# Quyans/GOI-Hyperplane

Hardware: AMD Instinct MI355X
Metric: training views/sec (rasterizer fwd+bwd), 1M Gaussians @1600x1056 RGB+16-d feat (higher is better)
Workload: dtype f32

## Files before the change

goi_hyperplane_amd/build.py:

```python
from __future__ import annotations

import os
import subprocess
import sys
from concurrent.futures import ThreadPoolExecutor

HERE = os.path.dirname(os.path.abspath(__file__))
ROOT = os.path.dirname(HERE)
CSRC = os.path.join(HERE, "csrc")
LIBDIR = os.path.join(HERE, "lib")
LIB = os.path.join(LIBDIR, "libgoi_raster.so")
HIPCC = os.environ.get("HIPCC", "/opt/rocm/bin/hipcc")
ARCH = "gfx950"

COMMON = ["--offload-arch=" + ARCH] + os.environ.get("GOI_EXTRA_FLAGS", "").split() + ["-O3", "-std=c++17", "-fPIC", "-I" + os.path.join(ROOT, "include"), "-I" + CSRC,
          "-munsafe-fp-atomics", "-Wall", "-Wno-unused-function"]
UNITS = {
    "api.hip": [],
    "scan_sort.hip": [],
    "preprocess.hip": ["-ffp-contract=off"],
    "binning.hip": [],
    "reduce_rows.hip": [],
    "render_fwd.hip": ["-fno-slp-vectorize"],
    "blend_stats.hip": [],
    "render_bwd.hip": [],
    "render_bwd_tile.hip": [],
    "render_bwd_sem.hip": [],
    "semantic_head.hip": [],
    "knn.hip": ["-ffp-contract=off"],
    "adam.hip": ["-ffp-contract=off"],
    "codebook_loss.hip": [],
    "osh.hip": [],
    "dbscan.hip": ["-ffp-contract=off"],
    "masks.hip": [],
    "codebook_init.hip": [],
    "photometric.hip": [],
    "densify.hip": ["-ffp-contract=off"],
    "display.hip": ["-ffp-contract=off"],
    "pca.hip": ["-ffp-contract=off"],
    "field.hip": ["-ffp-contract=off"],
    "mesh.hip": ["-ffp-contract=off"],
    "texture.hip": ["-ffp-contract=off"],
    "edit.hip": ["-ffp-contract=off"],
}


EXT = os.path.join(LIBDIR, "_goi_C.so")
EXT_SRC = os.path.join(CSRC, "torch_binding.cpp")


def build_torch_binding(force: bool = False, verbose: bool = False) -> str:
    import sysconfig
    import torch
    hdr = os.path.join(ROOT, "include", "goi_raster.h")
    if not force and os.path.exists(EXT) and all(os.path.getmtime(f) <= os.path.getmtime(EXT) for f in (EXT_SRC, hdr, LIB)):
        return EXT
    tdir = os.path.dirname(torch.__file__)
    cmd = [os.environ.get("CXX", "g++"), "-O2", "-std=c++17", "-fPIC", "-shared", "-D__HIP_PLATFORM_AMD__=1",
           "-DUSE_ROCM=1", "-DTORCH_EXTENSION_NAME=_goi_C", "-DTORCH_API_INCLUDE_EXTENSION_H",
           f"-D_GLIBCXX_USE_CXX11_ABI={int(torch._C._GLIBCXX_USE_CXX11_ABI)}",
           "-I" + os.path.join(tdir, "include"), "-I" + os.path.join(tdir, "include", "torch", "csrc", "api", "include"),
           "-I" + sysconfig.get_paths()["include"], "-I/opt/rocm/include", "-I" + os.path.join(ROOT, "include"),
           EXT_SRC, "-o", EXT, "-L" + os.path.join(tdir, "lib"), "-ltorch", "-ltorch_cpu", "-ltorch_python", "-lc10",
           "-lc10_hip", "-ltorch_hip", "-L" + LIBDIR, "-lgoi_raster", "-Wl,-rpath,$ORIGIN"]
    if verbose:
        print(" ".join(cmd))
    subprocess.check_call(cmd)
    return EXT


def _newer(src: str, dst: str) -> bool:
    return (not os.path.exists(dst)) or os.path.getmtime(src) > os.path.getmtime(dst)


def build(force: bool = False, verbose: bool = False) -> str:
    os.makedirs(LIBDIR, exist_ok=True)
    objdir = os.path.join(HERE, "build")
    os.makedirs(objdir, exist_ok=True)
    headers = [os.path.join(CSRC, h) for h in os.listdir(CSRC) if h.endswith(".h")] + [
        os.path.join(ROOT, "include", "goi_raster.h")]
    hdr_time = max(os.path.getmtime(h) for h in headers)

    def compile_one(item):
        name, extra = item
        src = os.path.join(CSRC, name)
        obj = os.path.join(objdir, name + ".o")
        if force or _newer(src, obj) or hdr_time > os.path.getmtime(obj):
            cmd = [HIPCC] + COMMON + extra + ["-c", src, "-o", obj]
            if verbose:
                print(" ".join(cmd))
            subprocess.check_call(cmd)
            return obj, True
        return obj, False

    with ThreadPoolExecutor(max_workers=4) as ex:
        results = list(ex.map(compile_one, UNITS.items()))
    objs = [o for o, _ in results]
    if force or any(c for _, c in results) or not os.path.exists(LIB):
        cmd = [HIPCC, "--offload-arch=" + ARCH, "-shared", "-fPIC", "-o", LIB] + objs
        if verbose:
            print(" ".join(cmd))
        subprocess.check_call(cmd)
    try:
        build_torch_binding(force=force, verbose=verbose)
    except Exception as ex:
        import warnings
        if os.path.exists(EXT):
            os.remove(EXT)
        warnings.warn(f"the compiled torch binding (_goi_C.so) could not be built: {ex}; goi_hyperplane_amd._C falls back "
                      "to its ctypes binding of the same C ABI (same kernels, ~0.14 ms more host time per step)")
    return LIB


if __name__ == "__main__":
    print(build(force="--force" in sys.argv, verbose=True))
```

goi_hyperplane_amd/csrc/render_bwd.hip:

```cpp
#include "blend_common.h"

namespace goi {

namespace {


#if !defined(GOI_BWD_WAVES)
#define GOI_BWD_WAVES 4
#endif
#define GOI_BWD_LAUNCH_BOUNDS __launch_bounds__(64, (S4 <= 4 ? GOI_BWD_WAVES : 2))

#ifndef GOI_TSTRIDE
#define GOI_TSTRIDE 66
#endif
constexpr int GROUP = 8;
constexpr int BATCH = 32;
constexpr int TSTRIDE = GOI_TSTRIDE;

template <int S4>
struct BwdCfg {
    static constexpr int NF4 = 1 + S4;
    static constexpr int NSEM = 4 * S4;
    static constexpr int NCH = NSEM + 4;
    static constexpr int NB = (NSEM + 15) / 16;
};

template <int S4, bool F16, bool MASKS>
__global__ GOI_BWD_LAUNCH_BOUNDS void render_bwd_rows_k(
    const uint2* __restrict__ ranges, const uint32_t* __restrict__ point_list, int W, int H, int gx, int gy,
    int n_quads, int S, const GaussRec* __restrict__ rec, const float* __restrict__ semantics,
    const int* __restrict__ radii, const uint4* __restrict__ aux, const float* __restrict__ bg,
    const float* __restrict__ out_alpha, const uint32_t* __restrict__ n_contrib, const float* __restrict__ dL_dpix,
    const float* __restrict__ dL_dpixsem, const float* __restrict__ dL_dpixdepth, const float* __restrict__ dL_dalphas,
    float* __restrict__ rows, uint8_t* __restrict__ flags, int row_floats,
    const uint32_t* __restrict__ counters, const uint32_t* __restrict__ qorder,
    const unsigned long long* __restrict__ qmask0, const unsigned long long* __restrict__ qmask,
    const uint32_t* __restrict__ qcost) {
    using Cfg = BwdCfg<S4>;
    const bool cull = counters[COUNTER_CULL] != 0;
    constexpr int NF4 = Cfg::NF4, NSEM = Cfg::NSEM, NCH = Cfg::NCH, NB = Cfg::NB;
    __shared__ f32x4 s_geo[BATCH + GROUP];
    __shared__ f32x4 s_geo2[BATCH + GROUP];
    __shared__ float2 s_cen[BATCH + GROUP];
    __shared__ __attribute__((aligned(16))) float4 s_feat[BATCH * NF4];
    constexpr int TS = TSTRIDE;
    constexpr int T_BYTES = F16 ? F16_FLOATS * 4 : 2 * GROUP * TSTRIDE * 4;
    __shared__ __attribute__((aligned(16))) char s_traw[T_BYTES];
    float* const s_t = reinterpret_cast<float*>(s_traw);

    const QuadGeom t = quad_geom_of(qorder ? (int)qorder[quad_slot()] : quad_slot(), W, H, gx, n_quads);
    if (t.tile < 0) return;
    if (counters[COUNTER_OVF]) return;
    const int lane = t.lane;
    const uint2 range = ranges[t.tile];
    const size_t HW = (size_t)W * H;
    const size_t pix_id = (size_t)W * t.py + t.px;
    const size_t pix_ld = t.inside ? pix_id : 0;
    const uint32_t nc_ld = n_contrib[pix_ld];
    const float oa_ld = out_alpha[pix_ld];
    float dLch[NCH];
    if (dL_dpixsem && S == NSEM) {
#pragma unroll
        for (int ch = 0; ch < NSEM; ch++) dLch[ch] = dL_dpixsem[ch * HW + pix_ld];
    } else {
#pragma unroll
        for (int ch = 0; ch < NSEM; ch++) dLch[ch] = (dL_dpixsem && ch < S) ? dL_dpixsem[ch * HW + pix_ld] : 0.f;
    }
    dLch[NSEM + 0] = dL_dpix ? dL_dpix[0 * HW + pix_ld] : 0.f;
    dLch[NSEM + 1] = dL_dpix ? dL_dpix[1 * HW + pix_ld] : 0.f;
    dLch[NSEM + 2] = dL_dpix ? dL_dpix[2 * HW + pix_ld] : 0.f;
    dLch[NSEM + 3] = dL_dpixdepth ? dL_dpixdepth[pix_ld] : 0.f;
    float dLa = dL_dalphas ? dL_dalphas[pix_ld] : 0.f;

    const int last_contributor = t.inside ? (int)nc_ld : 0;
    const int n_proc = qcost ? (int)qcost[__builtin_amdgcn_readfirstlane(4 * t.tile + t.q)] : wave_max_i32(last_contributor);
    if (n_proc == 0) return;
    const int rounds = (n_proc + BATCH - 1) / BATCH;

    const float T_final = t.inside ? (1.f - oa_ld) : 0.f;
    float T = T_final;
    if (!t.inside) {
#pragma unroll
        for (int ch = 0; ch < NCH; ch++) dLch[ch] = 0.f;
        dLa = 0.f;
    }
    const float bg_dot = bg[0] * dLch[NSEM] + bg[1] * dLch[NSEM + 1] + bg[2] * dLch[NSEM + 2];
    float R = 0.f;
    f32x2 dL2[NCH / 2];
#pragma unroll
    for (int i = 0; i < NCH / 2; i++) dL2[i] = f32x2{dLch[2 * i], dLch[2 * i + 1]};
    const f32x4* s_feat4 = reinterpret_cast<const f32x4*>(s_feat);

    const int kq = lane >> 4, mm = lane & 15;
    float bfrag[F16 ? 1 : NB][F16 ? 1 : 16];
    float bmix[F16 ? 1 : 16];
    f16x8 Wh[F16 ? NB : 1][2], Wl[F16 ? NB : 1][2], Cc[2];
    float unscale[F16 ? NB : 1], unscale_c = 0.f;
    bf16x8 Bas;
    constexpr int BT = 17;
    static_assert(64 * BT * 4 <= F16_FLOATS * 4 && 64 * 16 * 4 <= T_BYTES, "staging region too small");
    const float k1 = mm == 4 ? 1.f : 0.f, ku = mm == 5 ? 1.f : 0.f, kv = mm == 6 ? 1.f : 0.f;
    const float kuu = mm == 7 ? 1.f : 0.f, kuv = mm == 8 ? 1.f : 0.f, kvv = mm == 9 ? 1.f : 0.f;
    auto basis = [&](int p) {
        const float u = (float)(p & 7) - 3.5f, v = (float)(p >> 3) - 3.5f;
        return k1 + ku * u + kv * v + kuu * (u * u) + kuv * (u * v) + kvv * (v * v);
    };
    if constexpr (F16) {
#pragma unroll
        for (int nb = 0; nb < NB; nb++) {
#pragma unroll
            for (int c = 0; c < 16; c++) {
                const int ch = nb * 16 + c;
                s_t[lane * BT + c] = ch < NSEM ? dLch[ch] : 0.f;
            }
            __builtin_amdgcn_wave_barrier();
            float y[2][8];
#pragma unroll
            for (int c2 = 0; c2 < 2; c2++)
#pragma unroll
                for (int i = 0; i < 8; i++) y[c2][i] = s_t[(32 * c2 + 8 * kq + i) * BT + mm];
            f16_b_operand(y, Wh[nb], Wl[nb], unscale[nb]);
            __builtin_amdgcn_wave_barrier();
        }
        {
#pragma unroll
            for (int c = 0; c < 4; c++) s_t[lane * 5 + c] = dLch[NSEM + c];
            __builtin_amdgcn_wave_barrier();
            float y[2][8];
#pragma unroll
            for (int c2 = 0; c2 < 2; c2++)
#pragma unroll
                for (int i = 0; i < 8; i++) y[c2][i] = s_t[(32 * c2 + 8 * kq + i) * 5 + (mm & 3)];
            f16x8 hi[2], lo[2];
            f16_b_operand(y, hi, lo, unscale_c);
            typedef uint32_t u32x4 __attribute__((ext_vector_type(4)));
#pragma unroll
            for (int c2 = 0; c2 < 2; c2++) {
                const u32x4 hu = __builtin_bit_cast(u32x4, hi[c2]), lu = __builtin_bit_cast(u32x4, lo[c2]);
                u32x4 cu;
#pragma unroll
                for (int i = 0; i < 4; i++) cu[i] = mm < 4 ? hu[i] : mm < 8 ? lu[i] : 0u;
                Cc[c2] = __builtin_bit_cast(f16x8, cu);
            }
            __builtin_amdgcn_wave_barrier();
        }
        {
            float y[8];
            const float vb = (float)kq - 1.5f;
#pragma unroll
            for (int i = 0; i < 8; i++) {
                const float u = (float)i - 3.5f;
                y[i] = mm == 0 ? 1.f : mm == 1 ? u : mm == 2 ? vb : mm == 3 ? u * u : mm == 4 ? u * vb : mm == 5 ? vb * vb : 0.f;
            }
            bf16x8 unused;
            split_pack8(y, Bas, unused);
        }
    } else {
#pragma unroll
        for (int nb = 0; nb < NB; nb++) {
#pragma unroll
            for (int c = 0; c < 16; c++) {
                const int ch = nb * 16 + c;
                s_t[lane * 16 + c] = ch < NSEM ? dLch[ch] : 0.f;
            }
            __builtin_amdgcn_wave_barrier();
#pragma unroll
            for (int s = 0; s < 16; s++) bfrag[nb][s] = s_t[(4 * s + kq) * 16 + mm];
            __builtin_amdgcn_wave_barrier();
        }
#pragma unroll
        for (int c = 0; c < 4; c++) s_t[lane * 4 + c] = dLch[NSEM + c];
        __builtin_amdgcn_wave_barrier();
#pragma unroll
        for (int s = 0; s < 16; s++) bmix[s] = mm < 4 ? s_t[(4 * s + kq) * 4 + mm] : basis(4 * s + kq);
        __builtin_amdgcn_wave_barrier();
    }
    auto uniform = [](float x) { return __int_as_float(__builtin_amdgcn_readfirstlane(__float_as_int(x))); };
    const float QCX = uniform(t.QX0 + 3.5f), QCY = uniform(t.QY0 + 3.5f);
    const f32x2 uv = {t.pxf - QCX, t.pyf - QCY};
    const float half_W = uniform(0.5f * W), half_H = uniform(0.5f * H);

    uint32_t id_n = 0;
    unsigned long long w_n = 0;
    float4 q0_n = make_float4(0, 0, 0, 0), q1_n = make_float4(1.f, 0.f, -1.f, -1.f);
    const int tile_u = __builtin_amdgcn_readfirstlane(t.tile), q_u = __builtin_amdgcn_readfirstlane(t.q);
    const uint32_t x0_u = (uint32_t)__builtin_amdgcn_readfirstlane((int)range.x);
    auto prefetch = [&](int b) {
        if constexpr (MASKS) {
            w_n = *member_mask_ptr(const_cast<unsigned long long*>(qmask0), const_cast<unsigned long long*>(qmask), tile_u, q_u,
                                   x0_u, b >> 1);
            const int pos = b * BATCH + lane;
            if (lane < BATCH && pos < n_proc) id_n = point_list[range.x + (uint32_t)pos];
        } else {
            const int k = b * BATCH + lane;
            q1_n.z = -1.f;
            if (lane < BATCH && k < n_proc) {
                id_n = point_list[range.x + (n_proc - 1 - k)];
                const float4* r4 = reinterpret_cast<const float4*>(rec + id_n);
                q0_n = r4[0];
                q1_n = r4[1];
            }
        }
    };
    prefetch(MASKS ? rounds - 1 : 0);

    int nslot = 0;
    unsigned long long jpack = 0;

    auto xrow = [](int rho) { return rho * 8 + 16 * (rho >> 3); };
    auto flush_group = [&](int cnt) {
        f32x4 acc[NB];
        f32x4 accx = {0.f, 0.f, 0.f, 0.f};
#pragma unroll
        for (int nb = 0; nb < NB; nb++) acc[nb] = f32x4{0.f, 0.f, 0.f, 0.f};
        __builtin_amdgcn_wave_barrier();
        if constexpr (F16) {
            const f32x4* wsrc = reinterpret_cast<const f32x4*>(s_t + f16_lane_offset(mm, kq));
            {
                const f32x4* src = wsrc + (f16_row(GROUP) - f16_row(0)) / 4;
                const f32x4 a0 = src[0], a1 = src[1];
                const float y[8] = {a0.x, a0.y, a0.z, a0.w, a1.x, a1.y, a1.z, a1.w};
                bf16x8 Hh, Hl, Ht;
                split3_pack8(y, Hh, Hl, Ht);
                accx = __builtin_amdgcn_mfma_f32_16x16x32_bf16(Ht, Bas, accx, 0, 0, 0);
                accx = __builtin_amdgcn_mfma_f32_16x16x32_bf16(Hl, Bas, accx, 0, 0, 0);
                accx = __builtin_amdgcn_mfma_f32_16x16x32_bf16(Hh, Bas, accx, 0, 0, 0);
            }
            f32x4 accc = {0.f, 0.f, 0.f, 0.f};
            {
                f16x8 A0, A1;
                f16_a_operands(wsrc, A0, A1);
#pragma unroll
                for (int nb = 0; nb < NB; nb++) {
                    acc[nb] = __builtin_amdgcn_mfma_f32_16x16x32_f16(A0, Wl[nb][0], acc[nb], 0, 0, 0);
                    acc[nb] = __builtin_amdgcn_mfma_f32_16x16x32_f16(A1, Wl[nb][1], acc[nb], 0, 0, 0);
                    acc[nb] = __builtin_amdgcn_mfma_f32_16x16x32_f16(A0, Wh[nb][0], acc[nb], 0, 0, 0);
                    acc[nb] = __builtin_amdgcn_mfma_f32_16x16x32_f16(A1, Wh[nb][1], acc[nb], 0, 0, 0);
                }
                accc = __builtin_amdgcn_mfma_f32_16x16x32_f16(A0, Cc[0], accc, 0, 0, 0);
                accc = __builtin_amdgcn_mfma_f32_16x16x32_f16(A1, Cc[1], accc, 0, 0, 0);
            }
            __builtin_amdgcn_wave_barrier();
            if (mm < 8) {
                float* xb = s_t + xrow(4 * kq) + mm;
#pragma unroll
                for (int r = 0; r < 4; r++) xb[8 * r] = accx[r];
            }
            f32x2 sem[NB];
#pragma unroll
            for (int nb = 0; nb < NB; nb++) sem[nb] = (acc[nb].xy + acc[nb].zw) * unscale[nb];
            f32x2 col = accc.xy + accc.zw;
            col.x += __int_as_float(__builtin_amdgcn_update_dpp(0, __float_as_int(col.x), 0x104, 0xF, 0xF, true));
            col.y += __int_as_float(__builtin_amdgcn_update_dpp(0, __float_as_int(col.y), 0x104, 0xF, 0xF, true));
            col *= unscale_c;
#pragma unroll
            for (int e = 0; e < 2; e++) {
                const int j = 2 * kq + e;
                if (j < cnt) {
                    const int idx = (int)((jpack >> (8 * j)) & 0xFF);
                    float* dst = rows + (size_t)__float_as_uint(s_geo2[idx].w) * row_floats;
#pragma unroll
                    for (int nb = 0; nb < NB; nb++) {
                        const int ch = nb * 16 + mm;
                        if (ch < NSEM) dst[ch] = sem[nb][e];
                    }
                    if (mm < 4) dst[NSEM + mm] = col[e];
                }
            }
        } else {
#pragma unroll
            for (int s = 0; s < 16; s++) {
                const float a = s_t[mm * TS + 4 * s + kq];
#pragma unroll
                for (int nb = 0; nb < NB; nb++)
                    acc[nb] = __builtin_amdgcn_mfma_f32_16x16x4f32(a, bfrag[nb][s], acc[nb], 0, 0, 0);
                accx = __builtin_amdgcn_mfma_f32_16x16x4f32(a, bmix[s], accx, 0, 0, 0);
            }
        }
        __builtin_amdgcn_wave_barrier();
#pragma unroll
        for (int r = 0; r < 4 && !F16; r++) {
            const int row = 4 * kq + r;
            if (row >= GROUP && mm >= 4 && mm < 12) s_t[(row - GROUP) * 8 + (mm - 4)] = accx[r];
            if (row < cnt) {
                const int idx = (int)((jpack >> (8 * row)) & 0xFF);
                float* dst = rows + (size_t)__float_as_uint(s_geo2[idx].w) * row_floats;
#pragma unroll
                for (int nb = 0; nb < NB; nb++) {
                    const int ch = nb * 16 + mm;
                    if (ch < NSEM) dst[ch] = acc[nb][r];
                }
                if (mm < 4) dst[NSEM + mm] = accx[r];
            }
        }
        __builtin_amdgcn_wave_barrier();
        if (lane < cnt) {
            const float4 m03 = *reinterpret_cast<const float4*>(&s_t[lane * 8]);
            const float2 m45 = *reinterpret_cast<const float2*>(&s_t[lane * 8 + 4]);
            const int idx = (int)((jpack >> (8 * lane)) & 0xFF);
            const f32x4 g = s_geo[idx];
            const f32x4 g2 = s_geo2[idx];
            const float2 cen = s_cen[idx];
            const uint32_t slot = __float_as_uint(g2.w);
            const float Dx = cen.x, Dy = cen.y;
            float ca, cb, cc, inv_o;
            coef_decode(g, g2, ca, cb, cc, inv_o);
            float m0, sx, sy, sxx, sxy, syy;
            auto shift = [&](const float4& a, const float2& b, float DX, float DY) {
                m0 += a.x;
                sx += DX * a.x - a.y;
                sy += DY * a.x - a.z;
                sxx += DX * DX * a.x - 2.f * DX * a.y + a.w;
                sxy += DX * DY * a.x - DX * a.z - DY * a.y + b.x;
                syy += DY * DY * a.x - 2.f * DY * a.z + b.y;
            };
            m0 = sx = sy = sxx = sxy = syy = 0.f;
            if constexpr (F16) {
                const int r1 = 4 * (lane >> 1) + (lane & 1);
                shift(*reinterpret_cast<const float4*>(&s_t[xrow(r1)]), *reinterpret_cast<const float2*>(&s_t[xrow(r1) + 4]), Dx, Dy + 2.f);
                shift(*reinterpret_cast<const float4*>(&s_t[xrow(r1 + 2)]), *reinterpret_cast<const float2*>(&s_t[xrow(r1 + 2) + 4]), Dx, Dy - 2.f);
            } else {
                shift(m03, m45, Dx, Dy);
            }
            float* dst = rows + (size_t)slot * row_floats + NCH;
            dst[0] = -half_W * (ca * sx + cb * sy);
            dst[1] = -half_H * (cc * sy + cb * sx);
            dst[2] = -0.5f * sxx;
            dst[3] = -0.5f * sxy;
            dst[4] = -0.5f * syy;
            dst[5] = m0 * inv_o;
            flags[slot] = 1;
        }
        __builtin_amdgcn_wave_barrier();
    };

    for (int bi = 0; bi < rounds; bi++) {
        const int b = MASKS ? rounds - 1 - bi : bi;
        const uint32_t id = id_n;
        float4 q0 = q0_n, q1 = q1_n;
        bool hit;
        unsigned long long m;
        if constexpr (MASKS) {
            const uint32_t mem = (uint32_t)__builtin_amdgcn_readfirstlane((int)(uint32_t)(w_n >> (32 * (b & 1))));
            m = mem;
            hit = lane < BATCH && ((mem >> lane) & 1u);
            if (bi + 1 < rounds) prefetch(b - 1);
        } else {
            hit = ellipse_hits_quadrant(q0.x, q0.y, q0.z, q0.w, q1.x, q1.y, q1.z, q1.w, t.QX0, t.QY0);
            if (bi + 1 < rounds) prefetch(b + 1);
            m = __ballot(hit);
        }
        if (m == 0) continue;
        if (hit) {
            const float4* r4 = reinterpret_cast<const float4*>(rec + id);
            const float* srow = semantics + (size_t)id * S;
            const bool rows_of_float4 = (S & 3) == 0;
            lds_dma16(r4 + 2, &s_feat[0]);
            if (rows_of_float4) {
#pragma unroll
                for (int i = 0; i < S4; i++)
                    lds_dma16(reinterpret_cast<const float4*>(srow) + i, &s_feat[(1 + i) * BATCH]);
            }
            if constexpr (MASKS) {
                q0 = r4[0];
                q1 = r4[1];
            }
            int x0, y0, x1, y1;
            const uint4 ax = aux[id];
            listed_rect(q0.x, q0.y, (int)ax.y, q1.z, q1.w, cull, gx, gy, x0, y0, x1, y1);
            const uint32_t inst = ax.x + tile_instance(aux_mask(ax), t.tx, t.ty, x0, y0, x1);
            const PolyCoef pc = poly_coefs(q0.x, q0.y, q0.z, q0.w, q1.x, q1.y, QCX, QCY);
            int sl = lane;
            asm volatile("" : "+v"(sl));
            s_geo[sl] = f32x4{pc.A35.x, pc.A35.y, pc.A12.x, pc.A12.y};
            s_geo2[sl] = f32x4{pc.A0, pc.A4, pc.lim, __uint_as_float(inst * 4u + (uint32_t)t.q)};
            s_cen[sl] = make_float2(q0.x - QCX, q0.y - QCY);
            if (!rows_of_float4) {
#pragma unroll
                for (int i = 0; i < S4; i++) {
                    float4 v;
                    v.x = (4 * i + 0 < S) ? srow[4 * i + 0] : 0.f;
                    v.y = (4 * i + 1 < S) ? srow[4 * i + 1] : 0.f;
                    v.z = (4 * i + 2 < S) ? srow[4 * i + 2] : 0.f;
                    v.w = (4 * i + 3 < S) ? srow[4 * i + 3] : 0.f;
                    s_feat[(1 + i) * BATCH + sl] = v;
                }
            }
        }
        __builtin_amdgcn_s_waitcnt(0x0F70);
        __builtin_amdgcn_wave_barrier();

        while (m) {
            int j, pos0;
            if constexpr (MASKS) {
                j = 31 - __builtin_clz((uint32_t)m);
                m &= ~(1ull << j);
                pos0 = b * BATCH + j;
            } else {
                j = __builtin_ctzll(m);
                m &= m - 1;
                pos0 = n_proc - 1 - (b * BATCH + j);
            }
            const f32x4 g = s_geo[j];
            const f32x4 g2 = s_geo2[j];
            const PairEval e = eval_poly(g.xy, g.zw, g2.x, g2.y, g2.z, uv);
            const bool live = pos0 < last_contributor;
            if constexpr (!MASKS)
                if (!any_all(live, e.below, e.seen)) continue;
            const bool c = live && e.hit;

            const f32x4 f0 = s_feat4[j];
            f32x2 da = f0.xy * dL2[NSEM / 2];
            f32x2 db = f0.zw * dL2[NSEM / 2 + 1];
#pragma unroll
            for (int i = 0; i < S4; i++) {
                const f32x4 f = s_feat4[(1 + i) * BATCH + j];
                da = __builtin_elementwise_fma(f.xy, dL2[2 * i], da);
                db = __builtin_elementwise_fma(f.zw, dL2[2 * i + 1], db);
            }
            const f32x2 dot2 = da + db;
            const float dotv = (dot2.x + dot2.y) + dLa;
            const float one_m_a = 1.f - e.alpha;
            const float inv = __builtin_amdgcn_rcpf(one_m_a);
            const float Tn = T * inv;
            float wgt = 0.f, hval = 0.f;
            if (c) {
                const float dL_dopa = (dotv - R) * Tn - (T_final * inv) * bg_dot;
                R = e.alpha * dotv + one_m_a * R;
                T = Tn;
                wgt = e.alpha * Tn;
                hval = e.E * dL_dopa;
            }
            if constexpr (F16) {
                const int wrow = nslot * 72 + ((nslot & 1) << 2);
                s_t[wrow + lane] = wgt;
                s_t[wrow + lane + (f16_row(GROUP) - f16_row(0))] = hval;
            } else {
                s_t[nslot * TS + lane] = wgt;
                s_t[(GROUP + nslot) * TS + lane] = hval;
            }
            jpack |= (unsigned long long)j << (8 * nslot);
            nslot++;
            if (nslot == GROUP) {
                flush_group(GROUP);
                nslot = 0;
                jpack = 0;
            }
        }
        __builtin_amdgcn_wave_barrier();
        if (nslot > 0 && bi + 1 < rounds) {
            const int idx = (int)((jpack >> (8 * (lane & 7))) & 0xFF);
            if (lane < nslot) {
                s_geo[BATCH + lane] = s_geo[idx];
                s_geo2[BATCH + lane] = s_geo2[idx];
                s_cen[BATCH + lane] = s_cen[idx];
            }
            constexpr unsigned long long CARRY = 0x0706050403020100ull + 0x0101010101010101ull * BATCH;
            jpack = CARRY & ((1ull << (8 * nslot)) - 1ull);
            __builtin_amdgcn_wave_barrier();
        }
    }
    if (nslot > 0) flush_group(nslot);
}

constexpr int QO_THREADS = 1024, QO_WAVES = QO_THREADS / 64, QO_BUCKETS = 64, QO_ROUNDS = 16;
constexpr int QO_CLEAR_BLOCKS = 248;
__global__ __launch_bounds__(QO_THREADS) void quad_order_k(const uint32_t* __restrict__ qcost, int n_quads, int per,
                                                           uint32_t* __restrict__ qorder, int shift,
                                                           uint8_t* __restrict__ clear_flags,
                                                           const uint32_t* __restrict__ n_dev, uint32_t cap,
                                                           uint32_t* __restrict__ clear_ctl) {
    if (blockIdx.x >= 8) {
        if (clear_ctl && blockIdx.x == 8 && threadIdx.x < 8) clear_ctl[threadIdx.x] = 0u;
        if (!clear_flags) return;
        const size_t nq = ((size_t)min(*n_dev, cap) * 4 + 15) / 16;
        uint4* dst = reinterpret_cast<uint4*>(clear_flags);
        for (size_t i = (size_t)(blockIdx.x - 8) * QO_THREADS + threadIdx.x; i < nq; i += (size_t)QO_CLEAR_BLOCKS * QO_THREADS)
            dst[i] = make_uint4(0u, 0u, 0u, 0u);
        return;
    }
    __shared__ uint32_t cnt[QO_WAVES][QO_BUCKETS];
    const int band = blockIdx.x, base = band * per;
    const int n = max(0, min(per, n_quads - base));
    const int lane = threadIdx.x & 63, w = threadIdx.x >> 6;
    for (int i = threadIdx.x; i < QO_WAVES * QO_BUCKETS; i += QO_THREADS) (&cnt[0][0])[i] = 0;
    __syncthreads();
    const int chunk = (per + QO_WAVES - 1) / QO_WAVES;
    const unsigned long long lt = (1ull << lane) - 1ull;
    uint32_t d_r[QO_ROUNDS], rank_r[QO_ROUNDS];
#pragma unroll
    for (int r = 0; r < QO_ROUNDS; r++) {
        if (r * 64 >= chunk) break;
        const int e = w * chunk + r * 64 + lane;
        const bool ok = r * 64 + lane < chunk && e < n;
        const uint32_t c = ok ? qcost[base + e] : 0u;
        const uint32_t d = (uint32_t)(QO_BUCKETS - 1) - min((uint32_t)(QO_BUCKETS - 1), c >> shift);
        unsigned long long peers = __ballot(ok);
#pragma unroll
        for (int b = 0; b < 6; b++) {
            const bool bit = (d >> b) & 1u;
            const unsigned long long bal = __ballot(bit);
            peers &= bit ? bal : ~bal;
        }
        const uint32_t prev = ok ? cnt[w][d] : 0u;
        const uint32_t below = (uint32_t)__popcll(peers & lt);
        d_r[r] = d;
        rank_r[r] = prev + below;
        __builtin_amdgcn_wave_barrier();
        if (ok && below == 0) cnt[w][d] = prev + (uint32_t)__popcll(peers);
        __builtin_amdgcn_wave_barrier();
    }
    __syncthreads();
    if (threadIdx.x < 64) {
        uint32_t tot = 0;
        for (int ww = 0; ww < QO_WAVES; ww++) tot += cnt[ww][lane];
        uint32_t incl = tot;
#pragma unroll
        for (int dd = 1; dd < 64; dd <<= 1) {
            const uint32_t o = __shfl_up(incl, dd, 64);
            if (lane >= dd) incl += o;
        }
        uint32_t run = incl - tot;
        for (int ww = 0; ww < QO_WAVES; ww++) {
            const uint32_t t = cnt[ww][lane];
            cnt[ww][lane] = run;
            run += t;
        }
    }
    __syncthreads();
#pragma unroll
    for (int r = 0; r < QO_ROUNDS; r++) {
        const int e = w * chunk + r * 64 + lane;
        if (r * 64 + lane < chunk && e < n) qorder[base + cnt[w][d_r[r]] + rank_r[r]] = (uint32_t)(base + e);
    }
    for (int i = n + threadIdx.x; i < per; i += QO_THREADS) qorder[base + i] = 0xFFFFFFFFu;
}

template <int S4>
void launch_bwd_rows_s4(const GoiRasterScene& sc, const GeomView& g, const ImageView& im, const uint32_t* point_list,
                        const int* radii, const float* out_alpha, const PixelGrads& dpix, const BwdScratchView& scr,
                        bool exact_flush, bool walk_masks, hipStream_t s, const unsigned long long* qmask) {
    const int gx = (sc.W + TILE - 1) / TILE, gy = (sc.H + TILE - 1) / TILE;
    const int n_quads = gx * gy * 4;
#define GOI_LAUNCH_ROWS(F16, MASKS)                                                                                    \
    render_bwd_rows_k<S4, F16, MASKS><<<dim3(quad_grid(n_quads)), dim3(64), 0, s>>>(                                     \
        im.ranges, point_list, sc.W, sc.H, gx, gy, n_quads, sc.S, g.rec, sc.semantics, radii, g.aux, sc.bg, out_alpha, \
        im.n_contrib, dpix.color, dpix.semantic, dpix.depth, dpix.alpha, scr.rows, scr.flags, bwd_row_floats(sc.S),    \
        g.counters, quad_order_enabled(sc.W, sc.H) ? im.qorder : nullptr, im.qmask0, qmask, im.qcost)
    const bool masks = qmask != nullptr && walk_masks;
    if (exact_flush) {
        if (masks) GOI_LAUNCH_ROWS(false, true);
        else GOI_LAUNCH_ROWS(false, false);
    } else {
        if (masks) GOI_LAUNCH_ROWS(true, true);
        else GOI_LAUNCH_ROWS(true, false);
    }
#undef GOI_LAUNCH_ROWS
}

}

bool quad_order_enabled(int W, int H) {
    const int gx = (W + TILE - 1) / TILE, gy = (H + TILE - 1) / TILE;
    const int per = quad_grid(gx * gy * 4) / 8;
    return g_options.bwd_order != 0 && (per + QO_WAVES - 1) / QO_WAVES <= 64 * QO_ROUNDS;
}

bool launch_quad_order(const GoiRasterScene& sc, const ImageView& im, hipStream_t s, uint8_t* clear_flags,
                       const uint32_t* n_dev, uint32_t cap, uint32_t* clear_ctl) {
    if (!quad_order_enabled(sc.W, sc.H)) return false;
    const int gx = (sc.W + TILE - 1) / TILE, gy = (sc.H + TILE - 1) / TILE;
    const int n_quads = gx * gy * 4, per = quad_grid(n_quads) / 8;
    quad_order_k<<<dim3(clear_flags ? 8 + QO_CLEAR_BLOCKS : 8), dim3(QO_THREADS), 0, s>>>(
        im.qcost, n_quads, per, im.qorder, 3 + g_options.bwd_order, clear_flags, n_dev, cap, clear_ctl);
    return true;
}

void launch_render_bwd_rows(const GoiRasterScene& sc, const GeomView& g, const ImageView& im, const uint32_t* point_list,
                            const int* radii, const float* out_alpha, const PixelGrads& dpix, const BwdScratchView& scr,
                            bool exact_flush, bool walk_masks, hipStream_t s, const unsigned long long* qmask) {
#define GOI_CALL(N) launch_bwd_rows_s4<N>(sc, g, im, point_list, radii, out_alpha, dpix, scr, exact_flush, walk_masks, s, qmask)
    GOI_DISPATCH_S4(sc.S, GOI_CALL)
#undef GOI_CALL
}

}
```

goi_hyperplane_amd/csrc/render_fwd.hip:

```cpp
#include "blend_common.h"

namespace goi {

namespace {

template <int S4, bool TRACE, bool UNROLL2, bool MASKS, bool LEARN = false>
__global__ __launch_bounds__(64) void render_fwd_k(const uint2* __restrict__ ranges,
                                                   const uint32_t* __restrict__ point_list, int W, int H, int gx,
                                                   int n_quads, int S, const GaussRec* __restrict__ rec,
                                                   const float* __restrict__ semantics, const float* __restrict__ bg,
                                                   float* __restrict__ out_color, float* __restrict__ out_sem,
                                                   float* __restrict__ out_depth, float* __restrict__ out_alpha,
                                                   uint32_t* __restrict__ n_contrib, const float* __restrict__ img_sem,
                                                   float* __restrict__ gau_sem, int* __restrict__ num_gsem,
                                                   uint32_t* __restrict__ qcost, unsigned long long* __restrict__ qmask0,
                                                   unsigned long long* __restrict__ qmask, const float* __restrict__ zcut,
                                                   uint32_t* __restrict__ zlearn, uint32_t* __restrict__ frame_flags,
                                                   uint32_t* __restrict__ host_words, uint32_t stamp) {
    constexpr int NF4 = TRACE ? 1 : 1 + S4;
    constexpr int NSEM = TRACE ? 0 : 4 * S4;
    __shared__ f32x4 s_geo[64];
    __shared__ f32x4 s_geo2[64];
    __shared__ float4 s_feat[64 * NF4];
    const f32x4* s_feat4 = reinterpret_cast<const f32x4*>(s_feat);
    __shared__ uint32_t s_id[TRACE ? 64 : 1];

    if (host_words && blockIdx.x == 0 && threadIdx.x < 32) {
        host_words[threadIdx.x] = (frame_flags - COUNTER_OVF)[threadIdx.x];
        __threadfence_system();
        if (threadIdx.x == 0 && stamp)
            __hip_atomic_store(&host_words[HOST_STAMP_WORD], stamp, __ATOMIC_RELEASE, __HIP_MEMORY_SCOPE_SYSTEM);
    }
    const QuadGeom t = quad_geom(W, H, gx, n_quads);
    if (t.tile < 0) return;
    const int tq = quad_slot();
    const uint2 range = ranges[t.tile];
    const float QCX = t.QX0 + 3.5f, QCY = t.QY0 + 3.5f;
    const f32x2 uv = {t.pxf - QCX, t.pyf - QCY};
    const int len = (int)(range.y - range.x);
    const int rounds = (len + 63) / 64;
    const size_t HW = (size_t)W * H;
    const size_t pix_id = (size_t)W * t.py + t.px;
    const int lane = t.lane;

    float T = 1.0f;
    float T_live = t.inside ? 1.0f : 0.0f;
    auto all_done = [&]() { return __builtin_amdgcn_ballot_w64(T_live != 0.0f) == 0; };
    uint32_t last_contributor = 0;
    uint32_t stop_pos = 0;
    f32x2 C2[2] = {{0.f, 0.f}, {0.f, 0.f}};
    f32x2 Cs2[NSEM > 0 ? NSEM / 2 : 1];
#pragma unroll
    for (int i = 0; i < NSEM / 2; i++) Cs2[i] = f32x2{0.f, 0.f};

    uint32_t id_n = 0;
    float4 q0_n = make_float4(0, 0, 0, 0), q1_n = make_float4(1.f, 0.f, -1.f, -1.f), q2_n = make_float4(0, 0, 0, 0);
    auto prefetch = [&](int b) {
        const int k = b * 64 + lane;
        q1_n.z = -1.f;
        if (k < len) {
            id_n = point_list[range.x + k];
            const float4* r4 = reinterpret_cast<const float4*>(rec + id_n);
            q0_n = r4[0];
            q1_n = r4[1];
            q2_n = r4[2];
        }
    };
    if (rounds > 0) prefetch(0);

    const int tile_u = __builtin_amdgcn_readfirstlane(t.tile), q_u = __builtin_amdgcn_readfirstlane(t.q);
    const uint32_t x0_u = (uint32_t)__builtin_amdgcn_readfirstlane((int)range.x);
    auto store_members = [&](int b, unsigned long long mm) {
        if constexpr (MASKS)
            if (lane == 0) *member_mask_ptr(qmask0, qmask, tile_u, q_u, x0_u, b) = mm;
    };
    int b_end = rounds;
    for (int b = 0; b < rounds; b++) {
        if (all_done()) {
            b_end = b;
            break;
        }
        unsigned long long members = 0;
        const uint32_t id = id_n;
        const float4 q0 = q0_n, q1 = q1_n, q2 = q2_n;
        const bool hit = ellipse_hits_quadrant(q0.x, q0.y, q0.z, q0.w, q1.x, q1.y, q1.z, q1.w, t.QX0, t.QY0);
        if (b + 1 < rounds) prefetch(b + 1);
        unsigned long long m = __ballot(hit);
        if (m != 0 && hit) {
            const PolyCoef pc = poly_coefs(q0.x, q0.y, q0.z, q0.w, q1.x, q1.y, QCX, QCY);
            s_geo[lane] = f32x4{pc.A35.x, pc.A35.y, pc.A12.x, pc.A12.y};
            s_geo2[lane] = f32x4{pc.A0, pc.A4, pc.lim, 0.f};
            s_feat[lane * NF4] = q2;
            if constexpr (TRACE) {
                s_id[lane] = id;
            } else {
                const float* srow = semantics + (size_t)id * S;
                if ((S & 3) == 0) {
#pragma unroll
                    for (int i = 0; i < S4; i++) s_feat[lane * NF4 + 1 + i] = reinterpret_cast<const float4*>(srow)[i];
                } else {
#pragma unroll
                    for (int i = 0; i < S4; i++) {
                        float4 v;
                        v.x = (4 * i + 0 < S) ? srow[4 * i + 0] : 0.f;
                        v.y = (4 * i + 1 < S) ? srow[4 * i + 1] : 0.f;
                        v.z = (4 * i + 2 < S) ? srow[4 * i + 2] : 0.f;
                        v.w = (4 * i + 3 < S) ? srow[4 * i + 3] : 0.f;
                        s_feat[lane * NF4 + 1 + i] = v;
                    }
                }
            }
        }
        __builtin_amdgcn_wave_barrier();

        auto apply = [&](int j, const PairEval& e, bool valid) {
            const float test_T = T_live * (1.f - e.alpha);
            const bool c0 = valid && e.hit;
            const bool ok = test_T >= kTMin;
            const bool c = c0 && ok;
            const bool some = any_all(e.below, e.seen, ok);
            if (valid && some) {
                if constexpr (MASKS) asm("s_bitset1_b64 %0, %1" : "+s"(members) : "s"(j));
                const float wgt = c ? e.alpha * T_live : 0.f;
                const f32x2 w2 = {wgt, wgt};
                const f32x4 f0 = s_feat4[j * NF4];
                C2[0] = __builtin_elementwise_fma(f0.xy, w2, C2[0]);
                C2[1] = __builtin_elementwise_fma(f0.zw, w2, C2[1]);
                if constexpr (!TRACE) {
#pragma unroll
                    for (int i = 0; i < S4; i++) {
                        const f32x4 f = s_feat4[j * NF4 + 1 + i];
                        Cs2[2 * i] = __builtin_elementwise_fma(f.xy, w2, Cs2[2 * i]);
                        Cs2[2 * i + 1] = __builtin_elementwise_fma(f.zw, w2, Cs2[2 * i + 1]);
                    }
                } else {
                    if (c && (double)e.alpha > 0.005) {
                        const uint32_t gid = s_id[j];
                        for (int ch = 0; ch < S; ch++)
                            atomicAdd(&gau_sem[(size_t)gid * S + ch], img_sem[ch * HW + pix_id]);
                        atomicAdd(&num_gsem[gid], S);
                    }
                }
                if (c) {
                    T = test_T;
                    last_contributor = (uint32_t)(b * 64 + j + 1);
                }
            }
            if constexpr (LEARN)
                if (c0 && !ok) stop_pos = (uint32_t)(b * 64 + j + 1);
            T_live = c0 ? (ok ? test_T : 0.0f) : T_live;
        };
        if constexpr (UNROLL2) {
            while (m) {
                const int j0 = __builtin_ctzll(m);
                m &= m - 1;
                const bool has1 = m != 0;
                const int j1 = has1 ? __builtin_ctzll(m) : j0;
                if (has1) m &= m - 1;
                const f32x4 ga = s_geo[j0], gb = s_geo[j1];
                const f32x4 ha = s_geo2[j0], hb = s_geo2[j1];
                const PairEval e0 = eval_poly(ga.xy, ga.zw, ha.x, ha.y, ha.z, uv);
                const PairEval e1 = eval_poly(gb.xy, gb.zw, hb.x, hb.y, hb.z, uv);
                apply(j0, e0, true);
                apply(j1, e1, has1);
                if (all_done()) m = 0;
            }
        } else {
            while (m) {
                const int j = __builtin_ctzll(m);
                m &= m - 1;
                const f32x4 g = s_geo[j];
                const f32x4 g2 = s_geo2[j];
                const PairEval e = eval_poly(g.xy, g.zw, g2.x, g2.y, g2.z, uv);
                apply(j, e, true);
                if (all_done()) m = 0;
            }
        }
        store_members(b, members);
        __builtin_amdgcn_wave_barrier();
    }

    if constexpr (LEARN) {
        {
            const bool unsat = !all_done();
            const float zc_in = zcut ? zcut[tile_u] : __builtin_inff();
            float zc = __builtin_inff();
            if (unsat) {
                if (zc_in < 3.0e38f && lane == 0) atomicOr(frame_flags, OVF_CUT_TOO_TIGHT);
            } else {
                int seen = min(len, wave_max_i32((int)stop_pos));
                (void)b_end;
                if (zc_in < 3.0e38f && seen > 0) {
                    const float z_last = rec[point_list[range.x + (uint32_t)(seen - 1)]].q2.w;
                    if (z_last > zc_in && lane == 0) atomicOr(frame_flags, OVF_CUT_TOO_TIGHT);
                }
                const int pos = seen + (seen >> 3) + 32;
                if (pos < len)
                    zc = rec[point_list[range.x + (uint32_t)pos]].q2.w;
                else
                    zc = zc_in;
            }
            if (zlearn && lane == 0) atomicMax(&zlearn[tile_u], __float_as_uint(zc));
        }
    }

    {
        const int qc = wave_max_i32((int)last_contributor);
        if (qcost && lane == 0) qcost[tq] = (uint32_t)qc;
    }
    if (t.inside) {
        n_contrib[pix_id] = last_contributor;
        out_color[0 * HW + pix_id] = C2[0].x + T * bg[0];
        out_color[1 * HW + pix_id] = C2[0].y + T * bg[1];
        out_color[2 * HW + pix_id] = C2[1].x + T * bg[2];
        if constexpr (!TRACE) {
#pragma unroll
            for (int ch = 0; ch < NSEM; ch++)
                if (ch < S) out_sem[ch * HW + pix_id] = Cs2[ch >> 1][ch & 1];
            out_alpha[pix_id] = 1.f - T;
            out_depth[pix_id] = C2[1].y;
        }
    }
}


template <int S4>
void launch_fwd_s4(const GoiRasterScene& sc, const GeomView& g, const ImageView& im, const uint32_t* point_list,
                   float* out_color, float* out_sem, float* out_depth, float* out_alpha, hipStream_t s,
                   unsigned long long* qmask, const float* zcut, uint32_t* zlearn, uint32_t* host_words, uint32_t stamp) {
    const int gx = (sc.W + TILE - 1) / TILE, gy = (sc.H + TILE - 1) / TILE;
    const int n_quads = gx * gy * 4;
#define GOI_LAUNCH_FWD(U2, MK)                                                                                         \
    do {                                                                                                               \
        if (zlearn || zcut)     \
            render_fwd_k<S4, false, U2, MK, true><<<dim3(quad_grid(n_quads)), dim3(64), 0, s>>>(                        \
                im.ranges, point_list, sc.W, sc.H, gx, n_quads, sc.S, g.rec, sc.semantics, sc.bg, out_color, out_sem,   \
                out_depth, out_alpha, im.n_contrib, nullptr, nullptr, nullptr, im.qcost, im.qmask0, qmask, zcut,        \
                zlearn, g.counters + COUNTER_OVF, host_words, stamp);                                                   \
        else                                                                                                           \
            render_fwd_k<S4, false, U2, MK><<<dim3(quad_grid(n_quads)), dim3(64), 0, s>>>(                              \
                im.ranges, point_list, sc.W, sc.H, gx, n_quads, sc.S, g.rec, sc.semantics, sc.bg, out_color, out_sem,   \
                out_depth, out_alpha, im.n_contrib, nullptr, nullptr, nullptr, im.qcost, im.qmask0, qmask, zcut,        \
                zlearn, g.counters + COUNTER_OVF, host_words, stamp);                                                   \
    } while (0)
#ifdef GOI_FWD_NO_MASKS
    const bool masks = false;
#else
    const bool masks = qmask != nullptr;
#endif
    if (g_options.fwd_variant == 1) {
        if (masks) GOI_LAUNCH_FWD(true, true);
        else GOI_LAUNCH_FWD(true, false);
    } else {
        if (masks) GOI_LAUNCH_FWD(false, true);
        else GOI_LAUNCH_FWD(false, false);
    }
#undef GOI_LAUNCH_FWD
}

}

void launch_render_fwd(const GoiRasterScene& sc, const GeomView& g, const ImageView& im, const uint32_t* point_list,
                       float* out_color, float* out_sem, float* out_depth, float* out_alpha, hipStream_t s,
                       unsigned long long* qmask, const float* zcut, uint32_t* zlearn, uint32_t* host_words, uint32_t stamp) {
#define GOI_CALL(N) launch_fwd_s4<N>(sc, g, im, point_list, out_color, out_sem, out_depth, out_alpha, s, qmask, zcut, zlearn, host_words, stamp)
    GOI_DISPATCH_S4(sc.S, GOI_CALL)
#undef GOI_CALL
}

void launch_trace_fwd(const GoiRasterScene& sc, const float* img_sem, const GeomView& g, const ImageView& im,
                      const uint32_t* point_list, float* out_color, float* gau_sem, int* num_gsem, hipStream_t s) {
    const int gx = (sc.W + TILE - 1) / TILE, gy = (sc.H + TILE - 1) / TILE;
    const int n_quads = gx * gy * 4;
    render_fwd_k<1, true, false, false><<<dim3(quad_grid(n_quads)), dim3(64), 0, s>>>(
        im.ranges, point_list, sc.W, sc.H, gx, n_quads, sc.S, g.rec, nullptr, sc.bg, out_color, nullptr, nullptr, nullptr,
        im.n_contrib, img_sem, gau_sem, num_gsem, nullptr, nullptr, nullptr, nullptr, nullptr, g.counters + COUNTER_OVF,
        nullptr, 0u);
}

}
```

Measured before the change: 803.5.

## Interleave forward shared-memory records and make per-pixel termination checks uniform

The forward rasterizer's separate shared arrays for geometry, coefficients and features are merged into one interleaved per-Gaussian record. The apply step now branches on wave-uniform ballot masks, and the live-pixel ballot is recomputed only when some pixel terminates, instead of after every pair. Separately, the backward kernel pins FMA contraction explicitly in its moment-shift and opacity-gradient arithmetic and is compiled with SLP vectorization disabled. These changes target divergent branching, redundant ballots and scattered LDS reads, at the cost of extra ballot instructions per Gaussian and possible LDS bank conflicts from the strided record layout.

```diff
diff --git a/goi_hyperplane_amd/build.py b/goi_hyperplane_amd/build.py
--- a/goi_hyperplane_amd/build.py
+++ b/goi_hyperplane_amd/build.py
@@ -23,7 +23,7 @@
     "reduce_rows.hip": [],
     "render_fwd.hip": ["-fno-slp-vectorize"],
     "blend_stats.hip": [],
-    "render_bwd.hip": [],
+    "render_bwd.hip": ["-fno-slp-vectorize"],
     "render_bwd_tile.hip": [],
     "render_bwd_sem.hip": [],
     "semantic_head.hip": [],
diff --git a/goi_hyperplane_amd/csrc/render_bwd.hip b/goi_hyperplane_amd/csrc/render_bwd.hip
--- a/goi_hyperplane_amd/csrc/render_bwd.hip
+++ b/goi_hyperplane_amd/csrc/render_bwd.hip
@@ -307,12 +307,13 @@
             coef_decode(g, g2, ca, cb, cc, inv_o);
             float m0, sx, sy, sxx, sxy, syy;
             auto shift = [&](const float4& a, const float2& b, float DX, float DY) {
+#pragma clang fp contract(off)
                 m0 += a.x;
-                sx += DX * a.x - a.y;
-                sy += DY * a.x - a.z;
-                sxx += DX * DX * a.x - 2.f * DX * a.y + a.w;
-                sxy += DX * DY * a.x - DX * a.z - DY * a.y + b.x;
-                syy += DY * DY * a.x - 2.f * DY * a.z + b.y;
+                sx += __builtin_fmaf(DX, a.x, -a.y);
+                sy += __builtin_fmaf(DY, a.x, -a.z);
+                sxx += __builtin_fmaf(-(2.f * DX), a.y, (DX * DX) * a.x) + a.w;
+                sxy += __builtin_fmaf(-DY, a.y, __builtin_fmaf(DX * DY, a.x, -(DX * a.z))) + b.x;
+                syy += ((DY * DY) * a.x - (2.f * DY) * a.z) + b.y;
             };
             m0 = sx = sy = sxx = sxy = syy = 0.f;
             if constexpr (F16) {
@@ -425,8 +426,9 @@
             const float Tn = T * inv;
             float wgt = 0.f, hval = 0.f;
             if (c) {
-                const float dL_dopa = (dotv - R) * Tn - (T_final * inv) * bg_dot;
-                R = e.alpha * dotv + one_m_a * R;
+#pragma clang fp contract(off)
+                const float dL_dopa = __builtin_fmaf(-bg_dot, T_final * inv, (dotv - R) * Tn);
+                R = one_m_a * R + e.alpha * dotv;
                 T = Tn;
                 wgt = e.alpha * Tn;
                 hval = e.E * dL_dopa;
diff --git a/goi_hyperplane_amd/csrc/render_fwd.hip b/goi_hyperplane_amd/csrc/render_fwd.hip
--- a/goi_hyperplane_amd/csrc/render_fwd.hip
+++ b/goi_hyperplane_amd/csrc/render_fwd.hip
@@ -19,10 +19,9 @@
                                                    uint32_t* __restrict__ host_words, uint32_t stamp) {
     constexpr int NF4 = TRACE ? 1 : 1 + S4;
     constexpr int NSEM = TRACE ? 0 : 4 * S4;
-    __shared__ f32x4 s_geo[64];
-    __shared__ f32x4 s_geo2[64];
-    __shared__ float4 s_feat[64 * NF4];
-    const f32x4* s_feat4 = reinterpret_cast<const f32x4*>(s_feat);
+    constexpr int REC4 = NF4 + 2;
+    __shared__ float4 s_rec[64 * REC4];
+    const f32x4* s_rec4 = reinterpret_cast<const f32x4*>(s_rec);
     __shared__ uint32_t s_id[TRACE ? 64 : 1];
 
     if (host_words && blockIdx.x == 0 && threadIdx.x < 32) {
@@ -43,9 +42,10 @@
     const size_t pix_id = (size_t)W * t.py + t.px;
     const int lane = t.lane;
 
-    float T = 1.0f;
     float T_live = t.inside ? 1.0f : 0.0f;
-    auto all_done = [&]() { return __builtin_amdgcn_ballot_w64(T_live != 0.0f) == 0; };
+    float T_end = 1.0f;
+    unsigned long long live = __builtin_amdgcn_ballot_w64(T_live != 0.0f);
+    auto all_done = [&]() { return live == 0; };
     uint32_t last_contributor = 0;
     uint32_t stop_pos = 0;
     f32x2 C2[2] = {{0.f, 0.f}, {0.f, 0.f}};
@@ -88,16 +88,17 @@
         unsigned long long m = __ballot(hit);
         if (m != 0 && hit) {
             const PolyCoef pc = poly_coefs(q0.x, q0.y, q0.z, q0.w, q1.x, q1.y, QCX, QCY);
-            s_geo[lane] = f32x4{pc.A35.x, pc.A35.y, pc.A12.x, pc.A12.y};
-            s_geo2[lane] = f32x4{pc.A0, pc.A4, pc.lim, 0.f};
-            s_feat[lane * NF4] = q2;
+            float4* slot = s_rec + lane * REC4;
+            slot[0] = make_float4(pc.A35.x, pc.A35.y, pc.A12.x, pc.A12.y);
+            slot[1] = make_float4(pc.A0, pc.A4, pc.lim, 0.f);
+            slot[2] = q2;
             if constexpr (TRACE) {
                 s_id[lane] = id;
             } else {
                 const float* srow = semantics + (size_t)id * S;
                 if ((S & 3) == 0) {
 #pragma unroll
-                    for (int i = 0; i < S4; i++) s_feat[lane * NF4 + 1 + i] = reinterpret_cast<const float4*>(srow)[i];
+                    for (int i = 0; i < S4; i++) slot[3 + i] = reinterpret_cast<const float4*>(srow)[i];
                 } else {
 #pragma unroll
                     for (int i = 0; i < S4; i++) {
@@ -106,49 +107,56 @@
                         v.y = (4 * i + 1 < S) ? srow[4 * i + 1] : 0.f;
                         v.z = (4 * i + 2 < S) ? srow[4 * i + 2] : 0.f;
                         v.w = (4 * i + 3 < S) ? srow[4 * i + 3] : 0.f;
-                        s_feat[lane * NF4 + 1 + i] = v;
+                        slot[3 + i] = v;
                     }
                 }
             }
         }
         __builtin_amdgcn_wave_barrier();
 
-        auto apply = [&](int j, const PairEval& e, bool valid) {
+        auto apply = [&](const f32x4* r, int j, const PairEval& e) {
             const float test_T = T_live * (1.f - e.alpha);
-            const bool c0 = valid && e.hit;
             const bool ok = test_T >= kTMin;
-            const bool c = c0 && ok;
-            const bool some = any_all(e.below, e.seen, ok);
-            if (valid && some) {
+            const unsigned long long hm = __builtin_amdgcn_ballot_w64(e.below) & __builtin_amdgcn_ballot_w64(e.seen);
+            const unsigned long long om = __builtin_amdgcn_ballot_w64(ok);
+            if ((hm & om) != 0) {
                 if constexpr (MASKS) asm("s_bitset1_b64 %0, %1" : "+s"(members) : "s"(j));
-                const float wgt = c ? e.alpha * T_live : 0.f;
-                const f32x2 w2 = {wgt, wgt};
-                const f32x4 f0 = s_feat4[j * NF4];
-                C2[0] = __builtin_elementwise_fma(f0.xy, w2, C2[0]);
-                C2[1] = __builtin_elementwise_fma(f0.zw, w2, C2[1]);
-                if constexpr (!TRACE) {
-#pragma unroll
-                    for (int i = 0; i < S4; i++) {
-                        const f32x4 f = s_feat4[j * NF4 + 1 + i];
-                        Cs2[2 * i] = __builtin_elementwise_fma(f.xy, w2, Cs2[2 * i]);
-                        Cs2[2 * i + 1] = __builtin_elementwise_fma(f.zw, w2, Cs2[2 * i + 1]);
+                if (e.hit && ok) {
+                    const float wgt = e.alpha * T_live;
+                    const f32x2 w2 = {wgt, wgt};
+                    const f32x4 f0 = r[2];
+                    C2[0] = __builtin_elementwise_fma(f0.xy, w2, C2[0]);
+                    C2[1] = __builtin_elementwise_fma(f0.zw, w2, C2[1]);
+                    if constexpr (!TRACE) {
+#pragma unroll
+                        for (int i = 0; i < S4; i++) {
+                            const f32x4 f = r[3 + i];
+                            Cs2[2 * i] = __builtin_elementwise_fma(f.xy, w2, Cs2[2 * i]);
+                            Cs2[2 * i + 1] = __builtin_elementwise_fma(f.zw, w2, Cs2[2 * i + 1]);
+                        }
+                    } else {
+                        if ((double)e.alpha > 0.005) {
+                            const uint32_t gid = s_id[j];
+                            for (int ch = 0; ch < S; ch++)
+                                atomicAdd(&gau_sem[(size_t)gid * S + ch], img_sem[ch * HW + pix_id]);
+                            atomicAdd(&num_gsem[gid], S);
+                        }
                     }
-                } else {
-                    if (c && (double)e.alpha > 0.005) {
-                        const uint32_t gid = s_id[j];
-                        for (int ch = 0; ch < S; ch++)
-                            atomicAdd(&gau_sem[(size_t)gid * S + ch], img_sem[ch * HW + pix_id]);
-                        atomicAdd(&num_gsem[gid], S);
-                    }
-                }
-                if (c) {
-                    T = test_T;
+                    T_live = test_T;
                     last_contributor = (uint32_t)(b * 64 + j + 1);
                 }
             }
+            const unsigned long long em = hm & ~om;
             if constexpr (LEARN)
-                if (c0 && !ok) stop_pos = (uint32_t)(b * 64 + j + 1);
-            T_live = c0 ? (ok ? test_T : 0.0f) : T_live;
+                if (em != 0 && e.hit && !ok) stop_pos = (uint32_t)(b * 64 + j + 1);
+            if ((em & live) != 0) {
+                if (e.hit && !ok && T_live != 0.0f) {
+                    T_end = T_live;
+                    T_live = 0.0f;
+                }
+                live = __builtin_amdgcn_ballot_w64(T_live != 0.0f);
+                if (live == 0) m = 0;
+            }
         };
         if constexpr (UNROLL2) {
             while (m) {
@@ -157,23 +165,23 @@
                 const bool has1 = m != 0;
                 const int j1 = has1 ? __builtin_ctzll(m) : j0;
                 if (has1) m &= m - 1;
-                const f32x4 ga = s_geo[j0], gb = s_geo[j1];
-                const f32x4 ha = s_geo2[j0], hb = s_geo2[j1];
+                const f32x4 *ra = s_rec4 + j0 * REC4, *rb = s_rec4 + j1 * REC4;
+                const f32x4 ga = ra[0], gb = rb[0];
+                const f32x4 ha = ra[1], hb = rb[1];
                 const PairEval e0 = eval_poly(ga.xy, ga.zw, ha.x, ha.y, ha.z, uv);
                 const PairEval e1 = eval_poly(gb.xy, gb.zw, hb.x, hb.y, hb.z, uv);
-                apply(j0, e0, true);
-                apply(j1, e1, has1);
-                if (all_done()) m = 0;
+                apply(ra, j0, e0);
+                if (has1) apply(rb, j1, e1);
             }
         } else {
             while (m) {
                 const int j = __builtin_ctzll(m);
                 m &= m - 1;
-                const f32x4 g = s_geo[j];
-                const f32x4 g2 = s_geo2[j];
+                const f32x4* r = s_rec4 + j * REC4;
+                const f32x4 g = r[0];
+                const f32x4 g2 = r[1];
                 const PairEval e = eval_poly(g.xy, g.zw, g2.x, g2.y, g2.z, uv);
-                apply(j, e, true);
-                if (all_done()) m = 0;
+                apply(r, j, e);
             }
         }
         store_members(b, members);
@@ -209,6 +217,7 @@
         if (qcost && lane == 0) qcost[tq] = (uint32_t)qc;
     }
     if (t.inside) {
+        const float T = T_live != 0.0f ? T_live : T_end;
         n_contrib[pix_id] = last_contributor;
         out_color[0 * HW + pix_id] = C2[0].x + T * bg[0];
         out_color[1 * HW + pix_id] = C2[0].y + T * bg[1];
```

Result: faster. 826.5, median of 6 (+2.9%).
